# yondonfu/ai-rtc-agent

Measured on NVIDIA H100. Metric: frames/sec at 512x512 SD-Turbo img2img (1-step, stream-batch 1), higher is better.
Workload: dtype f16

## Files before the change

ai-rtc-agent_b200/csrc/capi.cu:

```cuda
#include "../../include/b200sd.h"

#include "attention.cuh"
#include "codec.cuh"
#include "elementwise.cuh"
#include "igemm.cuh"
#include "tconv.cuh"

using namespace b2;

extern "C" {

const char* b2sd_last_error(void) { return b2_last_error(); }
int b2sd_version(void) { return 1; }

static ActView to_view(const b2sd_act_view& v) {
    ActView a;
    a.ptr = reinterpret_cast<const __half*>(v.ptr);
    a.N = v.n; a.H = v.h; a.W = v.w; a.C = v.c; a.ld = v.ld;
    return a;
}

static void to_igemm_desc(const b2sd_igemm_desc* d, IgemmDesc& g) {
    g.nseg = d->nseg;
    for (int s = 0; s < d->nseg && s < IG_MAX_SRC; ++s) {
// ... 7 lines not shown
    g.Nb = d->nb; g.Ho = d->ho; g.Wo = d->wo;
    g.BN = d->bn;
    g.swap = d->swap;
    g.pair = (d->flags & B2SD_IG_PAIR) ? 1 : 0;
    g.splits = d->splits;
    g.partial = nullptr;
    g.dbg_ts = reinterpret_cast<unsigned long long*>(d->partial);
    g.epi.out = reinterpret_cast<__half*>(d->out);
    g.epi.ldc = d->ldc;
    g.epi.colbias = d->colbias;
    g.epi.colbias_bstride = d->colbias_bstride;
    g.epi.res = reinterpret_cast<const __half*>(d->res);
    g.epi.ldr = d->ldr;
    g.epi.acc_scale = d->acc_scale;
    g.epi.res_scale = d->res_scale;
    g.epi.flags = d->flags & (IG_RELU | IG_GEGLU | IG_SILU | IG_PAD0);
    g.epi.n_valid = d->n_valid;
    g.epi.rowstat_out = static_cast<unsigned long long*>(d->rowstat_out);
    g.epi.rowstat_in = static_cast<const unsigned long long*>(d->rowstat_in);
    g.epi.colsum = d->colsum;
    g.epi.ln_inv_c = d->ln_c > 0 ? 1.f / (float)d->ln_c : 0.f;
    g.epi.ln_eps = d->ln_eps;
    g.epi.out2 = reinterpret_cast<__half*>(d->out2);
    g.epi.ld2 = d->ld2;
    g.epi.col2 = d->col2;
}

static b2sd_act_view from_view(const ActView& a) {
    b2sd_act_view v;
    v.ptr = a.ptr;
    v.n = a.N; v.h = a.H; v.w = a.W; v.c = a.C; v.ld = a.ld;
// ... 3 lines not shown
static void fill_plan_info(const IgemmPlan& plan, b2sd_igemm_plan_info* out) {
    out->mode = plan.mode;
    out->swap = plan.p.swap;
    out->bn = plan.p.BN;
    out->splits = plan.splits;
    out->grid_x = (int)plan.grid.x; out->grid_y = (int)plan.grid.y; out->grid_z = (int)plan.grid.z;
    out->num_stages = plan.p.num_stages;
    out->acc_bufs = plan.p.acc_bufs;
    out->total_kb = plan.p.total_kb;
    out->kb_per_split = plan.p.kb_per_split;
    out->tmem_cols = (int)plan.p.tmem_cols;
    out->m_tiles = plan.p.tiles_w * plan.p.tiles_h * plan.p.tiles_n;
    out->smem_bytes = (int64_t)plan.smem;
    out->rows_total = plan.rows_total;
    out->tw = plan.p.tw; out->th = plan.p.th; out->tn = plan.p.tn;
}

}

namespace b2 {
void igemm_record(const IgemmDesc& g, const IgemmPlan* plan, b2sd_igemm_desc* d, b2sd_igemm_plan_info* info) {
    *d = b2sd_igemm_desc{};
    *info = b2sd_igemm_plan_info{};
    d->nseg = g.nseg;
    for (int s = 0; s < g.nseg && s < IG_MAX_SRC; ++s) {
        d->src[s] = from_view(g.src[s]);
        d->ntap[s] = g.ntap[s];
    }
    d->w = g.w;
    d->w_rows = g.w_rows;
// ... 227 lines not shown
```

ai-rtc-agent_b200/csrc/epilogue.cuh:

```cuda
#pragma once
#include "igemm.cuh"
#include "ptx.cuh"
#include "wgmma.cuh"

namespace b2 {

__device__ __forceinline__ float gelu_erf(float x) {
    return 0.5f * x * (1.0f + erff(x * 0.70710678118654752440f));
}

__device__ __forceinline__ float silu_f(float x) { return x / (1.0f + expf(-x)); }

__device__ __forceinline__ void store_half16(__half* dst, const float* v, int nv, bool vec_ok) {
    if (nv == 16 && vec_ok) {
        uint4 u[2];
        __half2* h = reinterpret_cast<__half2*>(u);
#pragma unroll
        for (int i = 0; i < 8; ++i) h[i] = __floats2half2_rn(v[2 * i], v[2 * i + 1]);
        reinterpret_cast<uint4*>(dst)[0] = u[0];
        reinterpret_cast<uint4*>(dst)[1] = u[1];
    } else {
#pragma unroll
        for (int i = 0; i < 16; ++i)
            if (i < nv) dst[i] = __float2half_rn(v[i]);
// ... 112 lines not shown
        *reinterpret_cast<__half2*>(dst) = __floats2half2_rn(x0, x1);
    } else {
        dst[0] = __float2half_rn(x0);
        if (two) dst[1] = __float2half_rn(x1);
    }
}

__device__ __forceinline__ void rowstat_quad(const IgEpilogue& e, const EpiRow& rw, float s1, float s2, int lane) {
    s1 += __shfl_xor_sync(0xffffffffu, s1, 1);
    s2 += __shfl_xor_sync(0xffffffffu, s2, 1);
    s1 += __shfl_xor_sync(0xffffffffu, s1, 2);
    s2 += __shfl_xor_sync(0xffffffffu, s2, 2);
    if ((lane & 3) == 0 && rw.ok) rowstat_add(e, rw.orow, s1, s2);
}

template <int BN, bool SILU = false>
__device__ __forceinline__ void epi_frag(const IgEpilogue& e, const float (&acc)[BN / 2], const EpiRow (&rw)[2], int ntile,
                                         bool ln_fma, int lane) {
    const int q2 = 2 * (lane & 3);
    const bool vec_out = (e.ldc & 1) == 0;
    if (e.flags & IG_GEGLU) {
        constexpr int HALF = BN / 2;
        const int pv0 = ntile * BN, oc0 = ntile * HALF;
#pragma unroll
        for (int j = 0; j < HALF / 8; ++j) {
            const int c = 8 * j + q2;
#pragma unroll
            for (int h = 0; h < 2; ++h) {
                if (!rw[h].ok) continue;
                float v[2];
#pragma unroll
                for (int u = 0; u < 2; ++u) {
                    float a = acc[4 * j + 2 * h + u], g = acc[4 * (j + HALF / 8) + 2 * h + u];
                    const int pv = pv0 + c + u, pg = pv0 + HALF + c + u;
                    if (ln_fma) {
                        const float nmr = -rw[h].mu * rw[h].rstd;
                        a = fmaf(rw[h].rstd, a, fmaf(nmr, e.colsum[pv], e.colbias ? e.colbias[pv] : 0.f));
                        g = fmaf(rw[h].rstd, g, fmaf(nmr, e.colsum[pg], e.colbias ? e.colbias[pg] : 0.f));
                    } else {
                        if (e.colsum) {
                            a = rw[h].rstd * (a - rw[h].mu * e.colsum[pv]);
                            g = rw[h].rstd * (g - rw[h].mu * e.colsum[pg]);
                        }
                        if (e.colbias) {
                            a += e.colbias[pv];
                            g += e.colbias[pg];
                        }
                    }
                    v[u] = a * gelu_erf(g);
                }
                store_half2(e.out + rw[h].orow * e.ldc + oc0 + c, v[0], v[1], true, vec_out);
            }
        }
        return;
    }
    float s1[2] = {0.f, 0.f}, s2[2] = {0.f, 0.f};
#pragma unroll
    for (int j = 0; j < BN / 8; ++j) {
        const int col = ntile * BN + 8 * j + q2;
        if (col >= e.n_valid) continue;
        const bool two = col + 1 < e.n_valid;
        const bool transposed = e.out2 && col >= e.col2;
#pragma unroll
        for (int h = 0; h < 2; ++h) {
            if (!rw[h].ok) continue;
            float x[2] = {acc[4 * j + 2 * h], acc[4 * j + 2 * h + 1]};
// ... 5 lines not shown
                    x[u] = fmaf(rw[h].rstd, x[u], fmaf(nmr, e.colsum[col + u], bp && (u == 0 || two) ? bp[u] : 0.f));
            } else {
                if (e.colsum) {
#pragma unroll
                    for (int u = 0; u < 2; ++u)
                        if (u == 0 || two) x[u] = rw[h].rstd * (x[u] - rw[h].mu * e.colsum[col + u]);
                }
                if (bp) {
                    x[0] += bp[0];
                    if (two) x[1] += bp[1];
                }
                if (e.acc_scale != 1.0f) {
                    x[0] *= e.acc_scale;
                    x[1] *= e.acc_scale;
                }
                if (e.res) {
                    const __half* rp = e.res + rw[h].orow * e.ldr + col;
                    if (two && (e.ldr & 1) == 0) {
                        const float2 f = __half22float2(*reinterpret_cast<const __half2*>(rp));
                        x[0] += e.res_scale * f.x;
                        x[1] += e.res_scale * f.y;
                    } else {
                        x[0] += e.res_scale * __half2float(rp[0]);
                        if (two) x[1] += e.res_scale * __half2float(rp[1]);
                    }
                }
                if (e.flags & IG_RELU) {
                    x[0] = fmaxf(x[0], 0.f);
                    x[1] = fmaxf(x[1], 0.f);
                }
                if (SILU && (e.flags & IG_SILU)) {
// ... 1 lines not shown
                    x[1] = silu_f(x[1]);
                }
            }
            if (transposed) {
                __half* tp = e.out2 + (long)(col - e.col2) * e.ld2 + rw[h].orow;
                tp[0] = __float2half_rn(x[0]);
                if (two) tp[e.ld2] = __float2half_rn(x[1]);
                continue;
            }
            if (e.rowstat_out && !ln_fma) {
                const float r0 = __half2float(__float2half_rn(x[0]));
                const float r1 = two ? __half2float(__float2half_rn(x[1])) : 0.f;
                s1[h] += r0 + r1;
                s2[h] += r0 * r0 + r1 * r1;
            }
            store_half2(e.out + rw[h].orow * e.ldc + col, x[0], x[1], two, vec_out);
        }
    }
    if (e.rowstat_out && !ln_fma) {
        rowstat_quad(e, rw[0], s1[0], s2[0], lane);
        rowstat_quad(e, rw[1], s1[1], s2[1], lane);
    }
}

template <int BN>
__device__ __forceinline__ void frag_to_smem(float* dst, const float (&acc)[BN / 2], int r0, int lane, int c0, int nc, bool colmajor) {
    const int q2 = 2 * (lane & 3);
#pragma unroll
    for (int j = 0; j < BN / 8; ++j) {
        const int c = 8 * j + q2 - c0;
        if (c < 0 || c >= nc) continue;
#pragma unroll
        for (int h = 0; h < 2; ++h) {
            const int r = r0 + 8 * h;
            if (colmajor) {
                dst[c * 128 + r] = acc[4 * j + 2 * h];
                dst[(c + 1) * 128 + r] = acc[4 * j + 2 * h + 1];
// ... 10 lines not shown
```

ai-rtc-agent_b200/csrc/igemm.cu:

```cuda
#include "igemm.cuh"

#include <cudaTypedefs.h>
#include <stdarg.h>
#include <stdio.h>
#include <stdlib.h>
#include <string.h>

#include "epilogue.cuh"
#include "launch.cuh"
#include "ptx.cuh"

namespace b2 {

#ifdef B2_TIMELINE
#define B2_TS(stmt) stmt
#else
#define B2_TS(stmt)
#endif

static thread_local char g_err[1024] = "";
const char* b2_last_error() { return g_err; }
void b2_set_error(const char* fmt, ...) {
    va_list ap;
    va_start(ap, fmt);
// ... 93 lines not shown
#pragma unroll
        for (int s = 0; s < G; ++s) {
            const uint32_t peer = dsmem_map(stg_local, (uint32_t)((s0 + s) * rank_mul + rank_add));
#pragma unroll
            for (int i = 0; i < 4; ++i) v[s][i] = dsmem_ld_f4(peer + (uint32_t)(((cc * 4 + i) * IG_BM + row) * 16));
        }
#pragma unroll
        for (int s = 0; s < G; ++s)
#pragma unroll
            for (int i = 0; i < 4; ++i) {
                acc[4 * i] += v[s][i].x; acc[4 * i + 1] += v[s][i].y; acc[4 * i + 2] += v[s][i].z; acc[4 * i + 3] += v[s][i].w;
            }
    }
}

template <int BN, bool PAIR, bool SILU, bool PAD0 = false>
__device__ __forceinline__ void igemm_body(const IgemmParams& p) {
    extern __shared__ uint8_t smem_raw[];
    uint8_t* smem = reinterpret_cast<uint8_t*>((reinterpret_cast<uintptr_t>(smem_raw) + 1023) &
                                               ~static_cast<uintptr_t>(1023));
    const int warp = threadIdx.x >> 5;
    const int lane = threadIdx.x & 31;
    constexpr uint32_t A_BYTES = IG_BM * IG_BK * 2;
    constexpr uint32_t stage_bytes = A_BYTES + (uint32_t)BN * IG_BK * 2;
    uint64_t* full_bar = reinterpret_cast<uint64_t*>(smem + (size_t)p.num_stages * stage_bytes);
    uint64_t* empty_bar = full_bar + IG_MAX_STAGES;
    const int cr = PAIR ? (int)(blockIdx.x & 1) : 0;
    const int mt_first = (int)blockIdx.x;
    const int mt_step = (int)gridDim.x;
    const int mt_guard = PAIR ? cr : 0;

    const int num_mtiles = p.tiles_w * p.tiles_h * p.tiles_n;
    const int ntile = blockIdx.y;
    const int kb_begin = blockIdx.z * p.kb_per_split;
    const int kb_end = min(p.total_kb, kb_begin + p.kb_per_split);
    [[maybe_unused]] unsigned long long* ts = p.dbg_ts ? p.dbg_ts + ((size_t)(blockIdx.z * gridDim.y + blockIdx.y) * gridDim.x + blockIdx.x) * 8 : nullptr;
    B2_TS(if (ts && threadIdx.x == 0) ts[0] = globaltimer_ns();)

    if (threadIdx.x == IG_CONS) {
        for (int s = 0; s < p.nseg; ++s) tma_prefetch_desc(&p.tmA[s]);
        tma_prefetch_desc(&p.tmB);
        for (int s = 0; s < p.num_stages; ++s) {
            mbar_init(&full_bar[s], 1);
            mbar_init(&empty_bar[s], (PAIR ? 2 : 1) * (IG_CONS / 32));
        }
        fence_mbar_init();
    }
    if (PAIR) {
        cluster_arrive_relaxed();
        cluster_wait();
    }
    __syncthreads();

    pdl_launch_dependents();
    pdl_wait();
    B2_TS(if (ts && threadIdx.x == 0) ts[1] = globaltimer_ns();)

    if (warp == IG_CONS / 32) {
        if (lane == 0) {
// ... 42 lines not shown
                        }
                    }
                    if (++stage == p.num_stages) {
                        stage = 0;
                        phase ^= 1;
                    }
                }
            }
        }
    } else {
        const int wg = warp >> 2;
        const int r0 = wg * 64 + (warp & 3) * 16 + (lane >> 2);
        [[maybe_unused]] const uint32_t peer_empty = PAIR ? dsmem_map(smem_u32(empty_bar), cluster_ctarank() ^ 1u) : 0u;
        const IgEpilogue& e = p.epi;
        const bool ln_fma = e.colsum && !p.swap && !(e.flags & IG_SPLITK) && (e.ldc & 7) == 0 && (e.n_valid & 15) == 0;
        const uint32_t smem_base = smem_u32(smem);
        auto release = [&](int s) {
            if (lane == 0) {
                mbar_arrive(&empty_bar[s]);
                if (PAIR) mbar_arrive_remote(peer_empty + (uint32_t)s * 8u);
            }
        };
        int stage = 0;
        uint32_t phase = 0;
        int it = 0;
        for (int mt = mt_first; mt - mt_guard < num_mtiles; mt += mt_step, ++it) {
            float acc[BN / 2];
#pragma unroll
            for (int i = 0; i < BN / 2; ++i) acc[i] = 0.f;
            int prev = -1;
// ... 5 lines not shown
                const uint64_t db = make_kmajor_sw128_desc(sa + A_BYTES);
#ifdef B2_BOUND_STUDY
                if (p.dbg_mode != 2)
#endif
                {
                    wgmma_fence_regs(acc);
                    wgmma_fence();
#pragma unroll
                    for (int k = 0; k < 4; ++k) Wgmma<BN>::ss(acc, da + 2 * k, db + 2 * k, 1u);
                    wgmma_commit();
                    wgmma_wait<1>();
                    wgmma_fence_regs(acc);
                }
                if (prev >= 0) release(prev);
                prev = stage;
                if (++stage == p.num_stages) {
                    stage = 0;
                    phase ^= 1;
                }
            }
            wgmma_wait<0>();
            wgmma_fence_regs(acc);
            if (prev >= 0) release(prev);
            B2_TS(if (ts && it == 0 && threadIdx.x == 0) ts[4] = globaltimer_ns();)

            const int w0 = (mt % p.tiles_w) * p.tw, h0 = ((mt / p.tiles_w) % p.tiles_h) * p.th;
            const int n0 = (mt / (p.tiles_w * p.tiles_h)) * p.tn;
            if (p.swap || (e.flags & IG_SPLITK)) {
                float* stg = reinterpret_cast<float*>(smem);
                cons_bar_sync();
// ... 9 lines not shown
                        cons_bar_sync();
                    }
                }
            } else {
                EpiRow rw[2];
#pragma unroll
                for (int h = 0; h < 2; ++h) {
                    const int r = r0 + 8 * h;
                    const int wi = r % p.tw, hi = (r / p.tw) % p.th, ni = r / (p.tw * p.th);
                    const int n = n0 + ni, hh = h0 + hi, ww = w0 + wi;
                    rw[h].ok = (ni < p.tn) && (n < p.Nb) && (hh < p.Ho) && (ww < p.Wo);
                    rw[h].orow = ((long)n * p.Ho + hh) * p.Wo + ww;
                    rw[h].b = n;
                    ln_row_stats(e, rw[h].orow, rw[h].ok, rw[h].mu, rw[h].rstd);
                }
                epi_frag<BN, SILU>(e, acc, rw, ntile, ln_fma, lane);
            }
            B2_TS(if (ts && it == 0 && threadIdx.x == 0) ts[5] = globaltimer_ns();)
        }
    }
    if (p.epi.flags & IG_SPLITK) {
        const int mt = blockIdx.x;
        const int w0 = (mt % p.tiles_w) * p.tw, h0 = ((mt / p.tiles_w) % p.tiles_h) * p.th;
        const int n0 = (mt / (p.tiles_w * p.tiles_h)) * p.tn;
        const int splits = (int)gridDim.z;
        const int rk_mul = PAIR ? 2 : 1, rk_add = cr;
        cluster_sync_all();
        B2_TS(if (ts && threadIdx.x == 0) ts[6] = globaltimer_ns();)
        if (warp < IG_CONS / 32 && p.swap) {
            const int rank = (int)cluster_ctarank();
            const int cols_per = BN / splits;
            const int ch = cols_per < SWAP_CH ? cols_per : SWAP_CH;
            const int t = threadIdx.x & (IG_BM - 1);
            const int half = threadIdx.x >> 7;
// ... 56 lines not shown
                    float mu, rstd;
                    ln_row_stats(p.epi, orow, true, mu, rstd);
                    epi_store16<0, 16, float, SILU>(p.epi, acc, n, orow, ntile * BN + cc * 16, mu, rstd);
                }
            }
        }
        B2_TS(if (ts && threadIdx.x == 0) ts[7] = globaltimer_ns();)
        cluster_sync_all();
    }
    if (PAIR) {
        cluster_arrive_relaxed();
        cluster_wait();
    }
}

template <int BN, bool PAIR, bool SILU = false>
__global__ void __launch_bounds__(IG_THREADS, 1) igemm_kernel(const __grid_constant__ IgemmParams p) { igemm_body<BN, PAIR, SILU>(p); }
template <int BN>
__global__ void __launch_bounds__(IG_THREADS, 1) igemm_pad0_kernel(const __grid_constant__ IgemmParams p) { igemm_body<BN, false, false, true>(p); }

using IgemmFn = void (*)(IgemmParams);
template <bool PAIR>
static IgemmFn igemm_fn(int bn) {
    switch (bn) {
#define B2_IG_CASE(N) case N: if constexpr (PAIR && (N % 32)) return nullptr; else return igemm_kernel<N, PAIR>;
        B2_IG_CASE(16) B2_IG_CASE(32) B2_IG_CASE(48) B2_IG_CASE(64) B2_IG_CASE(80) B2_IG_CASE(96) B2_IG_CASE(112) B2_IG_CASE(128)
        B2_IG_CASE(144) B2_IG_CASE(160) B2_IG_CASE(176) B2_IG_CASE(192) B2_IG_CASE(208) B2_IG_CASE(224) B2_IG_CASE(240) B2_IG_CASE(256)
#undef B2_IG_CASE
        default: return nullptr;
    }
}
static IgemmFn igemm_select(int bn, bool pair, bool silu, bool pad0 = false) {
    if (pad0) {
        if (pair || silu) return nullptr;
        switch (bn) {
            case 64: return igemm_pad0_kernel<64>;
            case 128: return igemm_pad0_kernel<128>;
            case 256: return igemm_pad0_kernel<256>;
            default: return nullptr;
        }
    }
    if (!silu) return pair ? igemm_fn<true>(bn) : igemm_fn<false>(bn);
    if (pair) return nullptr;
    switch (bn) {
        case 16: return igemm_kernel<16, false, true>;
        case 32: return igemm_kernel<32, false, true>;
        case 64: return igemm_kernel<64, false, true>;
// ... 9 lines not shown
    cudaDriverEntryPointQueryResult qres;
    cudaError_t err = cudaGetDriverEntryPoint("cuTensorMapEncodeTiled", &p, cudaEnableDefault, &qres);
    if (err != cudaSuccess || qres != cudaDriverEntryPointSuccess || !p) {
        b2_set_error("cudaGetDriverEntryPoint(cuTensorMapEncodeTiled) failed: %s",
                     cudaGetErrorString(err));
        return nullptr;
    }
    fn = reinterpret_cast<PFN_cuTensorMapEncodeTiled_v12000>(p);
    return fn;
}

static thread_local bool g_plan_dry = false;
void igemm_set_dry_run(bool on) { g_plan_dry = on; }

static int encode_act_map(CUtensorMap* m, const ActView& a, int box_c, int box_w, int box_h, int box_n,
                          int estride) {
    if (g_plan_dry) return 0;
    auto enc = get_encode();
    if (!enc) return -1;
    cuuint64_t dims[4] = {(cuuint64_t)a.C, (cuuint64_t)a.W, (cuuint64_t)a.H, (cuuint64_t)a.N};
    cuuint64_t strides[3] = {(cuuint64_t)a.ld * 2, (cuuint64_t)a.W * a.ld * 2,
                             (cuuint64_t)a.H * a.W * a.ld * 2};
    cuuint32_t box[4] = {(cuuint32_t)box_c, (cuuint32_t)box_w, (cuuint32_t)box_h, (cuuint32_t)box_n};
    cuuint32_t es[4] = {1, (cuuint32_t)estride, (cuuint32_t)estride, 1};
    CUresult r = enc(m, CU_TENSOR_MAP_DATA_TYPE_FLOAT16, 4, const_cast<__half*>(a.ptr), dims, strides,
                     box, es, CU_TENSOR_MAP_INTERLEAVE_NONE, CU_TENSOR_MAP_SWIZZLE_128B,
                     CU_TENSOR_MAP_L2_PROMOTION_L2_256B, CU_TENSOR_MAP_FLOAT_OOB_FILL_NONE);
    if (r != CUDA_SUCCESS) {
        b2_set_error("cuTensorMapEncodeTiled(act) failed: %d (ptr %p dims %d,%d,%d,%d ld %d box "
                     "%d,%d,%d,%d es %d)",
                     (int)r, a.ptr, a.C, a.W, a.H, a.N, a.ld, box_c, box_w, box_h, box_n, estride);
        return -1;
    }
    return 0;
}

static int encode_w_map(CUtensorMap* m, const __half* w, int rows, int ld, int box_rows) {
    if (g_plan_dry) return 0;
    auto enc = get_encode();
    if (!enc) return -1;
    cuuint64_t dims[2] = {(cuuint64_t)ld, (cuuint64_t)rows};
// ... 125 lines not shown
            sms = n;
        else
            sms = IG_SMS;
        cudaGetLastError();
    }
    return sms;
}

static int igemm_ctas_per_sm(int bn, bool pair, bool silu, bool pad0) {
    if (g_plan_dry) return 1;
    IgemmFn fn = igemm_select(bn, pair, silu, pad0);
    int n = 0;
    if (fn && cudaOccupancyMaxActiveBlocksPerMultiprocessor(&n, fn, IG_THREADS, 0) == cudaSuccess && n > 0) return n;
    cudaGetLastError();
    return 1;
}

int igemm_plan(const IgemmDesc& d, IgemmPlan* plan) {
    *plan = IgemmPlan{};
    if (d.swap) return plan_swap(d, plan);
    IgemmParams& p = plan->p;
    if (d.nseg < 1 || d.nseg > IG_MAX_SRC) {
        b2_set_error("igemm: bad nseg %d", d.nseg);
        return -1;
    }
    const bool geglu = (d.epi.flags & IG_GEGLU) != 0;
    const int n_gemm = geglu ? d.epi.n_valid * 2 : d.epi.n_valid;
    int BN = d.BN;
    if (BN <= 0) {
        if (n_gemm <= 256 && n_gemm % 16 == 0) BN = n_gemm;
// ... 125 lines not shown
    p.num_stages = stages;
    size_t pipe_bytes = stages * stage_bytes;
    if (splits > 1) {
        const size_t stg = (size_t)BN * IG_BM * 4;
        if (stg > pipe_bytes) {
            stages = (int)((stg + stage_bytes - 1) / stage_bytes);
            if (stages > IG_MAX_STAGES) {
                b2_set_error("igemm: split-K staging does not fit (BN %d)", BN);
                return -1;
            }
            p.num_stages = stages;
            pipe_bytes = stages * stage_bytes;
        }
    }
    plan->smem = pipe_bytes + 1024  + 512 ;
    const int m_tiles = p.tiles_w * p.tiles_h * p.tiles_n;
    int grid_x = m_tiles;
    p.acc_bufs = 1;
    if (will_persist) {
        grid_x = (int)(persist_ctas / n_tiles);
        if (grid_x < 1) grid_x = 1;
        if (grid_x > m_tiles) grid_x = m_tiles;
        p.acc_bufs = 2;
    }
    if (pair) {
        grid_x = (p.acc_bufs == 2 && grid_x > 2) ? (grid_x & ~1) : ((grid_x + 1) & ~1);
    }
    uint32_t cols = 32;
    while (cols < (uint32_t)(BN * p.acc_bufs)) cols <<= 1;
    p.tmem_cols = cols;
    plan->grid = dim3(grid_x, n_tiles, splits);
    plan->mode = pair ? 1 : 0;
    plan->pair = pair ? 1 : 0;
    return 0;
}

int igemm_encode_act_map(CUtensorMap* m, const ActView& a, int box_c, int box_w, int box_h, int box_n, int estride) {
    return encode_act_map(m, a, box_c, box_w, box_h, box_n, estride);
}
int igemm_encode_w_map(CUtensorMap* m, const __half* w, int rows, int ld, int box_rows) { return encode_w_map(m, w, rows, ld, box_rows); }

int igemm_init() {
    static bool attr_set = false;
    if (!attr_set) {
        for (int bn = 16; bn <= 256; bn += 16) {
            for (int pair = 0; pair < 4; ++pair) {
                IgemmFn fn = igemm_select(bn, pair == 1, pair == 2, pair == 3);
                if (!fn) continue;
                cudaError_t e = cudaFuncSetAttribute(fn, cudaFuncAttributeMaxDynamicSharedMemorySize, 227 * 1024);
                if (e != cudaSuccess) {
                    b2_set_error("cudaFuncSetAttribute(igemm BN %d%s): %s", bn, pair ? " pair" : "", cudaGetErrorString(e));
                    return -1;
                }
            }
        }
        if (!get_encode()) return -1;
        attr_set = true;
    }
    return 0;
}

int igemm_launch(const IgemmPlan& plan, cudaStream_t stream) {
    if (igemm_init()) return -1;
    const int cz = plan.splits > 1 ? plan.splits : 1;
    IgemmFn fn = igemm_select(plan.p.BN, plan.pair, (plan.p.epi.flags & IG_SILU) != 0, (plan.p.epi.flags & IG_PAD0) != 0);
    if (!fn) {
        b2_set_error("igemm launch: no kernel for BN %d%s%s%s", plan.p.BN, plan.pair ? " (CTA pair)" : "",
                     (plan.p.epi.flags & IG_SILU) ? " with the SiLU epilogue" : "", (plan.p.epi.flags & IG_PAD0) ? " with tap origin 0" : "");
        return -1;
    }
    cudaError_t e = plan.pair ? launch_kc(fn, plan.grid, dim3(IG_THREADS), plan.smem, stream, 2, cz, plan.p)
                              : launch_k(fn, plan.grid, dim3(IG_THREADS), plan.smem, stream, cz, plan.p);
    if (e != cudaSuccess) {
        b2_set_error("igemm launch: %s", cudaGetErrorString(e));
        return -1;
    }
    return 0;
}

}
// ... 1 lines not shown
```

ai-rtc-agent_b200/csrc/igemm.cuh:

```cuda
#pragma once
#include <cuda.h>
#include <cuda_fp16.h>
#include <cuda_runtime.h>
#include <stdint.h>

namespace b2 {

constexpr int IG_BM = 128;
constexpr int IG_BK = 64;
constexpr int IG_MAX_SRC = 3;
constexpr int IG_MAX_STAGES = 8;
constexpr int IG_CONS = 256;
constexpr int IG_THREADS = IG_CONS + 32;
constexpr int IG_SMS = 132;

enum : int {
    IG_RELU = 1,
    IG_GEGLU = 2,
    IG_SPLITK = 4,
    IG_SILU = 8,
    IG_PAD0 = 16,
};

struct IgEpilogue {
    __half* out;
    int ldc;
    const float* colbias;
    int colbias_bstride;
    const __half* res;
    int ldr;
    float acc_scale;
    float res_scale;
    int flags;
    int n_valid;
    unsigned long long* rowstat_out;
    const unsigned long long* rowstat_in;
    const float* colsum;
    float ln_inv_c, ln_eps;
    __half* out2;
    int ld2, col2;
};

constexpr float IG_STAT_SCALE = 1048576.f;

struct IgemmParams {
    CUtensorMap tmA[IG_MAX_SRC];
    CUtensorMap tmB;
    int seg_ntap[IG_MAX_SRC];
    int seg_cblocks[IG_MAX_SRC];
    int seg_c0[IG_MAX_SRC];
    int nseg;
    int total_kb;
    int kb_per_split;
    int tw, th, tn;
    int tiles_w, tiles_h, tiles_n;
    int Wo, Ho, Nb;
    int stride;
    int BN;
    int num_stages;
    int acc_bufs;
    uint32_t a_bytes;
    uint32_t b_bytes;
    uint32_t tmem_cols;
    unsigned long long* dbg_ts;
    int n_pad;
    int swap;
    int tw_log2, th_log2;
    int dbg_mode;
    IgEpilogue epi;
};

struct ActView {
    const __half* ptr;
    int N, H, W, C;
    int ld;
};

struct IgemmDesc {
    ActView src[IG_MAX_SRC];
    int ntap[IG_MAX_SRC];
    int nseg;
    const __half* w;
    int w_rows;
// ... 40 lines not shown
```

ai-rtc-agent_b200/host/capi.py:

```python
from __future__ import annotations

import ctypes as C
import os

_HERE = os.path.dirname(os.path.abspath(__file__))
LIB_PATH = os.environ.get("B200SD_LIB") or os.path.join(os.path.dirname(_HERE), "libb200sd.so")


class B2Error(RuntimeError):
    pass


class ActView(C.Structure):
    _fields_ = [("ptr", C.c_void_p), ("n", C.c_int), ("h", C.c_int), ("w", C.c_int), ("c", C.c_int),
                ("ld", C.c_int)]


class IgemmDesc(C.Structure):
    _fields_ = [
        ("src", ActView * 3), ("ntap", C.c_int * 3), ("nseg", C.c_int),
        ("w", C.c_void_p), ("w_rows", C.c_int), ("w_ld", C.c_int), ("stride", C.c_int),
        ("nb", C.c_int), ("ho", C.c_int), ("wo", C.c_int),
        ("bn", C.c_int), ("splits", C.c_int), ("partial", C.c_void_p),
        ("out", C.c_void_p), ("ldc", C.c_int),
# ... 1 lines not shown
        ("res", C.c_void_p), ("ldr", C.c_int),
        ("acc_scale", C.c_float), ("res_scale", C.c_float),
        ("flags", C.c_int), ("n_valid", C.c_int), ("swap", C.c_int),
        ("rowstat_out", C.c_void_p), ("rowstat_in", C.c_void_p), ("colsum", C.c_void_p), ("ln_c", C.c_int), ("ln_eps", C.c_float),
        ("out2", C.c_void_p), ("ld2", C.c_int), ("col2", C.c_int),
    ]


class IgemmPlanInfo(C.Structure):
    _fields_ = [
        ("mode", C.c_int), ("swap", C.c_int), ("bn", C.c_int), ("splits", C.c_int),
        ("grid_x", C.c_int), ("grid_y", C.c_int), ("grid_z", C.c_int),
        ("num_stages", C.c_int), ("acc_bufs", C.c_int), ("total_kb", C.c_int), ("kb_per_split", C.c_int),
        ("tmem_cols", C.c_int), ("m_tiles", C.c_int),
        ("smem_bytes", C.c_int64), ("rows_total", C.c_int64),
        ("tw", C.c_int), ("th", C.c_int), ("tn", C.c_int),
    ]


class AttnDesc(C.Structure):
    _fields_ = [
        ("q", C.c_void_p), ("ldq", C.c_int),
        ("k", C.c_void_p), ("ldk", C.c_int), ("k_bstride", C.c_int64), ("k_rows", C.c_int64),
        ("vt", C.c_void_p), ("ldvt", C.c_int), ("vt_bstride", C.c_int64), ("vt_cols", C.c_int64),
        ("out", C.c_void_p), ("ldo", C.c_int),
        ("nb", C.c_int), ("heads", C.c_int), ("sq", C.c_int), ("skv", C.c_int), ("d_real", C.c_int),
        ("dp", C.c_int),
    ]


class GroupNormArgs(C.Structure):
# ... 89 lines not shown
        ("vae", C.c_int), ("vae_scaling_factor", C.c_float),
    ]


class LoraFactor(C.Structure):
    _fields_ = [("key", C.c_char_p), ("up", C.c_void_p), ("down", C.c_void_p), ("rank", C.c_int), ("dtype", C.c_int),
                ("scale", C.c_float)]


IN_U8_NHWC, IN_F32_NCHW, IN_F16_NCHW = 0, 1, 2
OUT_U8_NCHW, OUT_F16_NCHW = 0, 1
IG_RELU = 1
IG_GEGLU = 2
IG_SILU = 8
IG_PAD0 = 16
SC_IN_U8, SC_IN_TANH3, SC_OUT_RELU, SC_OUT_SILU, SC_IN_OFFSET = 1, 2, 4, 32, 64
CONTROL_FRAME, CONTROL_HED = 0, 1
COND_PROMPT, COND_TIME = 0, 1
VAE_TINY, VAE_KL = 0, 1
IG_TCONV = 64
IG_PAIR = 128

_lib = None


def lib() -> C.CDLL:
    global _lib
    if _lib is None:
        if not os.path.exists(LIB_PATH):
            raise B2Error(f"{LIB_PATH} not found: build it with `make -C ai-rtc-agent_b200/csrc` "
# ... 91 lines not shown
```

ai-rtc-agent_b200/host/ops.py:

```python
from __future__ import annotations

import ctypes as C
from typing import Optional, Sequence, Tuple

import torch

from . import capi


_SCRATCH = {}


def pack_conv_weight(w_oihw: torch.Tensor) -> torch.Tensor:
    o, i, kh, kw = w_oihw.shape
    return w_oihw.permute(0, 2, 3, 1).reshape(o, kh * kw * i).contiguous().to(torch.float16)


def _pitch(t: torch.Tensor) -> int:
    n, h, w, _ = t.shape
    return t.stride(2) if w > 1 or (h == 1 and n == 1) else (t.stride(1) if h > 1 else t.stride(0))


def _view(t: torch.Tensor) -> capi.ActView:
    assert t.dtype == torch.float16 and t.is_cuda and t.dim() == 4
    n, h, w, c = t.shape
    assert t.stride(3) == 1 and t.stride(2) % 8 == 0
    ld = t.stride(2)
    assert t.stride(1) == w * ld and t.stride(0) == h * w * ld, "NHWC view must be dense in n,h,w"
    return capi.ActView(t.data_ptr(), n, h, w, c, ld)


def igemm(srcs: Sequence[Tuple[torch.Tensor, int]], w: torch.Tensor, out: torch.Tensor, *,
          stride: int = 1, colbias: Optional[torch.Tensor] = None, res: Optional[torch.Tensor] = None,
          acc_scale: float = 1.0, res_scale: float = 1.0, relu: bool = False, geglu: bool = False, silu: bool = False,
          bn: int = 0, splits: int = 1, n_valid: Optional[int] = None, timeline: Optional[torch.Tensor] = None, swap: bool = False,
          tconv: bool = False, pair: bool = False, pad0: bool = False,
          rowstat_out: Optional[torch.Tensor] = None, rowstat_in: Optional[torch.Tensor] = None,
          colsum: Optional[torch.Tensor] = None, ln_c: int = 0, ln_eps: float = 1e-5,
          out2: Optional[torch.Tensor] = None, col2: int = 0) -> torch.Tensor:
    d = _igemm_desc(srcs, w, out, stride=stride, colbias=colbias, res=res, acc_scale=acc_scale, res_scale=res_scale, relu=relu,
                    geglu=geglu, silu=silu, bn=bn, splits=splits, n_valid=n_valid, timeline=timeline, swap=swap, tconv=tconv, pair=pair,
                    pad0=pad0,
                    rowstat_out=rowstat_out, rowstat_in=rowstat_in, colsum=colsum, ln_c=ln_c, ln_eps=ln_eps, out2=out2, col2=col2)
    capi.check(capi.lib().b2sd_op_igemm(C.byref(d), capi.current_stream_ptr()), "b2sd_op_igemm")
    return out


def igemm_engine_plan(srcs, w, out, *, autotile: int = 1, allow_swap: bool = True, **kw) -> capi.IgemmPlanInfo:
    d = _igemm_desc(srcs, w, out, **kw)
    info = capi.IgemmPlanInfo()
    capi.check(capi.lib().b2sd_igemm_plan_dry(C.byref(d), autotile, int(allow_swap), C.byref(info)), "b2sd_igemm_plan_dry")
    return info


def _igemm_desc(srcs, w, out, *, stride=1, colbias=None, res=None, acc_scale=1.0, res_scale=1.0, relu=False, geglu=False,
                silu=False, bn=0, splits=1, n_valid=None, timeline=None, swap=False, tconv=False, pair=False, pad0=False, rowstat_out=None,
                rowstat_in=None, colsum=None, ln_c=0, ln_eps=1e-5, out2=None, col2=0) -> capi.IgemmDesc:
    d = capi.IgemmDesc()
    d.nseg = len(srcs)
    for i, (t, ntap) in enumerate(srcs):
        d.src[i] = _view(t)
        d.ntap[i] = ntap
    assert w.dtype == torch.float16 and w.is_contiguous()
    d.w, d.w_rows, d.w_ld = w.data_ptr(), w.shape[0], w.shape[1]
    d.stride = stride
    nb, ho, wo, _ = out.shape
    d.nb, d.ho, d.wo = nb, ho, wo
    d.bn, d.splits = bn, splits
    d.swap = int(swap)
    d.out, d.ldc = out.data_ptr(), _pitch(out)
    nv = n_valid if n_valid is not None else out.shape[3]
    d.n_valid = nv
    if timeline is not None:
        d.partial = timeline.data_ptr()
    if colbias is not None:
        assert colbias.dtype == torch.float32 and colbias.is_contiguous()
        d.colbias = colbias.data_ptr()
        d.colbias_bstride = colbias.shape[1] if colbias.dim() == 2 and colbias.shape[0] > 1 else 0
    if res is not None:
        assert res.dtype == torch.float16
        d.res, d.ldr = res.data_ptr(), _pitch(res)
    d.acc_scale, d.res_scale = acc_scale, res_scale
    d.flags = (capi.IG_RELU if relu else 0) | (capi.IG_GEGLU if geglu else 0) | (capi.IG_TCONV if tconv else 0) | (capi.IG_PAIR if pair else 0) \
        | (capi.IG_SILU if silu else 0) | (capi.IG_PAD0 if pad0 else 0)
    if rowstat_out is not None:
        assert rowstat_out.dtype == torch.int64 and rowstat_out.is_contiguous()
        d.rowstat_out = rowstat_out.data_ptr()
    if rowstat_in is not None:
        assert rowstat_in.dtype == torch.int64 and colsum is not None and colsum.dtype == torch.float32 and ln_c > 0
        d.rowstat_in, d.colsum, d.ln_c, d.ln_eps = rowstat_in.data_ptr(), colsum.data_ptr(), ln_c, ln_eps
    if out2 is not None:
        assert out2.dtype == torch.float16 and out2.dim() == 2 and out2.stride(1) == 1
        d.out2, d.ld2, d.col2 = out2.data_ptr(), out2.stride(0), col2
    return d


def _sp():
    return capi.current_stream_ptr()

# ... 105 lines not shown
```

include/b200sd.h:

```cpp
#ifndef B200SD_H
#define B200SD_H

#include <stdint.h>

#ifdef __cplusplus
extern "C" {
#endif

const char* b2sd_last_error(void);
int b2sd_version(void);


typedef struct {
    const void* ptr;
    int n, h, w, c;
    int ld;
} b2sd_act_view;

enum {
    B2SD_IG_RELU = 1,
    B2SD_IG_GEGLU = 2,
    B2SD_IG_SILU = 8,
    B2SD_IG_PAD0 = 16,
    B2SD_IG_TCONV = 64,
    B2SD_IG_PAIR = 128
};

typedef struct {
    b2sd_act_view src[3];
    int ntap[3];
    int nseg;
    const void* w;
    int w_rows, w_ld;
    int stride;
    int nb, ho, wo;
    int bn;
    int splits;
    void* partial;
// ... 17 lines not shown
} b2sd_igemm_desc;

int b2sd_op_igemm(const b2sd_igemm_desc* d, void* stream);

typedef struct {
    int mode;
    int swap, bn, splits;
    int grid_x, grid_y, grid_z;
    int num_stages;
    int acc_bufs;
    int total_kb, kb_per_split;
    int tmem_cols;
    int m_tiles;
    int64_t smem_bytes, rows_total;
    int tw, th, tn;
} b2sd_igemm_plan_info;
int b2sd_igemm_plan_dry(const b2sd_igemm_desc* d, int autotile, int allow_swap, b2sd_igemm_plan_info* out);

int b2sd_groupnorm_plan_dry(int ca, int cb, int groups, int hw, int* cluster, int* threads, int* pixels_per_cta);
uint64_t b2sd_igemm_partial_floats(int splits, int64_t rows_total, int n_valid);

typedef struct {
    const void* q; int ldq;
    const void* k; int ldk; int64_t k_bstride; int64_t k_rows;
    const void* vt; int ldvt; int64_t vt_bstride; int64_t vt_cols;
    void* out; int ldo;
    int nb, heads, sq, skv, d_real, dp;
} b2sd_attn_desc;
int b2sd_op_attention(const b2sd_attn_desc* d, void* stream);

// ... 180 lines not shown
```

Baseline: 197.6.

## Stage igemm epilogue through swizzled smem with TMA residual prefetch and store

Adds a staged epilogue to the implicit-GEMM kernel. At the first k-block the residual tile is prefetched into a 64B-swizzled shared-memory buffer by TMA. Results are then written to that buffer and sent out as bulk TMA stores, replacing per-thread scattered global half2 loads and stores. This needs extra shared memory, which can lower stages or occupancy, and more kernel template instantiations. Staging is on by default and is skipped for split-K, SiLU, pad0, and misaligned outputs.

Result: faster. 205.8 (median of 6 runs) (+4.2%).

```diff
diff --git a/ai-rtc-agent_b200/csrc/capi.cu b/ai-rtc-agent_b200/csrc/capi.cu
--- a/ai-rtc-agent_b200/csrc/capi.cu
+++ b/ai-rtc-agent_b200/csrc/capi.cu
@@ -45,7 +45,7 @@
     g.epi.ldr = d->ldr;
     g.epi.acc_scale = d->acc_scale;
     g.epi.res_scale = d->res_scale;
-    g.epi.flags = d->flags & (IG_RELU | IG_GEGLU | IG_SILU | IG_PAD0);
+    g.epi.flags = d->flags & (IG_RELU | IG_GEGLU | IG_SILU | IG_PAD0 | IG_NO_STAGE);
     g.epi.n_valid = d->n_valid;
     g.epi.rowstat_out = static_cast<unsigned long long*>(d->rowstat_out);
     g.epi.rowstat_in = static_cast<const unsigned long long*>(d->rowstat_in);
@@ -79,6 +79,7 @@
     out->smem_bytes = (int64_t)plan.smem;
     out->rows_total = plan.rows_total;
     out->tw = plan.p.tw; out->th = plan.p.th; out->tn = plan.p.tn;
+    out->staged = plan.p.staged;
 }
 
 }
diff --git a/ai-rtc-agent_b200/csrc/epilogue.cuh b/ai-rtc-agent_b200/csrc/epilogue.cuh
--- a/ai-rtc-agent_b200/csrc/epilogue.cuh
+++ b/ai-rtc-agent_b200/csrc/epilogue.cuh
@@ -150,11 +150,14 @@
     if ((lane & 3) == 0 && rw.ok) rowstat_add(e, rw.orow, s1, s2);
 }
 
-template <int BN, bool SILU = false>
+template <int BN, bool SILU = false, bool STAGED = false>
 __device__ __forceinline__ void epi_frag(const IgEpilogue& e, const float (&acc)[BN / 2], const EpiRow (&rw)[2], int ntile,
-                                         bool ln_fma, int lane) {
+                                         bool ln_fma, int lane, uint8_t* stg = nullptr) {
     const int q2 = 2 * (lane & 3);
     const bool vec_out = (e.ldc & 1) == 0;
+    auto sp = [&](int h, int j) {
+        return reinterpret_cast<__half2*>(stg + h * (8 * 64) + (j >> 2) * IG_STG_BOX + (((j & 3) ^ (lane >> 3)) << 4));
+    };
     if (e.flags & IG_GEGLU) {
         constexpr int HALF = BN / 2;
         const int pv0 = ntile * BN, oc0 = ntile * HALF;
@@ -185,7 +188,8 @@
                     }
                     v[u] = a * gelu_erf(g);
                 }
-                store_half2(e.out + rw[h].orow * e.ldc + oc0 + c, v[0], v[1], true, vec_out);
+                if constexpr (STAGED) *sp(h, j) = __floats2half2_rn(v[0], v[1]);
+                else store_half2(e.out + rw[h].orow * e.ldc + oc0 + c, v[0], v[1], true, vec_out);
             }
         }
         return;
@@ -221,7 +225,11 @@
                     x[0] *= e.acc_scale;
                     x[1] *= e.acc_scale;
                 }
-                if (e.res) {
+                if (STAGED && e.res) {
+                    const float2 f = __half22float2(*sp(h, j));
+                    x[0] += e.res_scale * f.x;
+                    x[1] += e.res_scale * f.y;
+                } else if (e.res) {
                     const __half* rp = e.res + rw[h].orow * e.ldr + col;
                     if (two && (e.ldr & 1) == 0) {
                         const float2 f = __half22float2(*reinterpret_cast<const __half2*>(rp));
@@ -253,13 +261,18 @@
                 s1[h] += r0 + r1;
                 s2[h] += r0 * r0 + r1 * r1;
             }
-            store_half2(e.out + rw[h].orow * e.ldc + col, x[0], x[1], two, vec_out);
+            if constexpr (STAGED) *sp(h, j) = __floats2half2_rn(x[0], x[1]);
+            else store_half2(e.out + rw[h].orow * e.ldc + col, x[0], x[1], two, vec_out);
         }
     }
     if (e.rowstat_out && !ln_fma) {
         rowstat_quad(e, rw[0], s1[0], s2[0], lane);
         rowstat_quad(e, rw[1], s1[1], s2[1], lane);
     }
+}
+
+__device__ __forceinline__ uint8_t* stg_thread(uint8_t* stg, int warp, int lane) {
+    return stg + ((warp & 3) * 16 + (lane >> 2)) * 64 + 4 * (lane & 3);
 }
 
 template <int BN>
diff --git a/ai-rtc-agent_b200/csrc/igemm.cu b/ai-rtc-agent_b200/csrc/igemm.cu
--- a/ai-rtc-agent_b200/csrc/igemm.cu
+++ b/ai-rtc-agent_b200/csrc/igemm.cu
@@ -131,17 +131,19 @@
     }
 }
 
-template <int BN, bool PAIR, bool SILU, bool PAD0 = false>
+template <int BN, bool PAIR, bool SILU, bool PAD0 = false, bool STAGED = false>
 __device__ __forceinline__ void igemm_body(const IgemmParams& p) {
     extern __shared__ uint8_t smem_raw[];
-    uint8_t* smem = reinterpret_cast<uint8_t*>((reinterpret_cast<uintptr_t>(smem_raw) + 1023) &
-                                               ~static_cast<uintptr_t>(1023));
+    uint8_t* smem = smem_raw + ((1024u - (smem_u32(smem_raw) & 1023u)) & 1023u);
     const int warp = threadIdx.x >> 5;
     const int lane = threadIdx.x & 31;
     constexpr uint32_t A_BYTES = IG_BM * IG_BK * 2;
     constexpr uint32_t stage_bytes = A_BYTES + (uint32_t)BN * IG_BK * 2;
-    uint64_t* full_bar = reinterpret_cast<uint64_t*>(smem + (size_t)p.num_stages * stage_bytes);
+    const uint32_t stg_bytes = STAGED ? (uint32_t)p.stg_boxes * IG_STG_BOX : 0u;
+    uint8_t* stg_base = smem + (size_t)p.num_stages * stage_bytes;
+    uint64_t* full_bar = reinterpret_cast<uint64_t*>(stg_base + 2 * stg_bytes);
     uint64_t* empty_bar = full_bar + IG_MAX_STAGES;
+    uint64_t* r_full = empty_bar + IG_MAX_STAGES;
     const int cr = PAIR ? (int)(blockIdx.x & 1) : 0;
     const int mt_first = (int)blockIdx.x;
     const int mt_step = (int)gridDim.x;
@@ -160,6 +162,12 @@
         for (int s = 0; s < p.num_stages; ++s) {
             mbar_init(&full_bar[s], 1);
             mbar_init(&empty_bar[s], (PAIR ? 2 : 1) * (IG_CONS / 32));
+        }
+        if (stg_bytes) {
+            tma_prefetch_desc(&p.tmO);
+            if (p.epi.res) tma_prefetch_desc(&p.tmR);
+            mbar_init(&r_full[0], 1);
+            mbar_init(&r_full[1], 1);
         }
         fence_mbar_init();
     }
@@ -232,6 +240,11 @@
         [[maybe_unused]] const uint32_t peer_empty = PAIR ? dsmem_map(smem_u32(empty_bar), cluster_ctarank() ^ 1u) : 0u;
         const IgEpilogue& e = p.epi;
         const bool ln_fma = e.colsum && !p.swap && !(e.flags & IG_SPLITK) && (e.ldc & 7) == 0 && (e.n_valid & 15) == 0;
+        const bool staged = stg_bytes && !(e.out2 && (ntile + 1) * BN > e.col2);
+        const bool leader = (threadIdx.x & 127) == 0;
+        const bool load_res = e.res && !(e.flags & IG_GEGLU) && !ln_fma;
+        const int ow = (e.flags & IG_GEGLU) ? BN / 2 : BN;
+        uint8_t* stg = stg_base + wg * stg_bytes;
         const uint32_t smem_base = smem_u32(smem);
         auto release = [&](int s) {
             if (lane == 0) {
@@ -267,6 +280,19 @@
                 }
                 if (prev >= 0) release(prev);
                 prev = stage;
+                if (staged && leader && kb == kb_begin) {
+                    const int w0 = (mt % p.tiles_w) * p.tw, h0 = ((mt / p.tiles_w) % p.tiles_h) * p.th;
+                    const int n0 = (mt / (p.tiles_w * p.tiles_h)) * p.tn;
+                    bulk_wait_group_read<0>();
+                    if (load_res) {
+                        mbar_expect_tx(&r_full[wg], stg_bytes);
+                        for (int b = 0; b < p.stg_boxes; ++b)
+                            tma_load_4d(stg + b * IG_STG_BOX, &p.tmR, &r_full[wg], ntile * ow + 32 * b, w0 + wg * p.stg_dw,
+                                        h0 + wg * p.stg_dh, n0 + wg * p.stg_dn);
+                    } else {
+                        mbar_arrive(&r_full[wg]);
+                    }
+                }
                 if (++stage == p.num_stages) {
                     stage = 0;
                     phase ^= 1;
@@ -306,10 +332,24 @@
                     rw[h].b = n;
                     ln_row_stats(e, rw[h].orow, rw[h].ok, rw[h].mu, rw[h].rstd);
                 }
-                epi_frag<BN, SILU>(e, acc, rw, ntile, ln_fma, lane);
+                if (staged) {
+                    mbar_wait(&r_full[wg], (uint32_t)it & 1u);
+                    epi_frag<BN, SILU, true>(e, acc, rw, ntile, ln_fma, lane, stg_thread(stg, warp, lane));
+                    fence_proxy_async_smem();
+                    named_bar_sync(2 + wg, 128);
+                    if (leader) {
+                        for (int b = 0; b < p.stg_boxes; ++b)
+                            tma_store_4d(&p.tmO, stg + b * IG_STG_BOX, ntile * ow + 32 * b, w0 + wg * p.stg_dw, h0 + wg * p.stg_dh,
+                                         n0 + wg * p.stg_dn);
+                        bulk_commit_group();
+                    }
+                } else {
+                    epi_frag<BN, SILU>(e, acc, rw, ntile, ln_fma, lane);
+                }
             }
             B2_TS(if (ts && it == 0 && threadIdx.x == 0) ts[5] = globaltimer_ns();)
         }
+        if (staged && leader) bulk_wait_group<0>();
     }
     if (p.epi.flags & IG_SPLITK) {
         const int mt = blockIdx.x;
@@ -396,23 +436,29 @@
     }
 }
 
-template <int BN, bool PAIR, bool SILU = false>
-__global__ void __launch_bounds__(IG_THREADS, 1) igemm_kernel(const __grid_constant__ IgemmParams p) { igemm_body<BN, PAIR, SILU>(p); }
+template <int BN, bool PAIR, bool SILU = false, bool STAGED = false>
+__global__ void __launch_bounds__(IG_THREADS, 1) igemm_kernel(const __grid_constant__ IgemmParams p) {
+    igemm_body<BN, PAIR, SILU, false, STAGED>(p);
+}
 template <int BN>
 __global__ void __launch_bounds__(IG_THREADS, 1) igemm_pad0_kernel(const __grid_constant__ IgemmParams p) { igemm_body<BN, false, false, true>(p); }
 
 using IgemmFn = void (*)(IgemmParams);
-template <bool PAIR>
+template <bool PAIR, bool STAGED = false>
 static IgemmFn igemm_fn(int bn) {
     switch (bn) {
-#define B2_IG_CASE(N) case N: if constexpr (PAIR && (N % 32)) return nullptr; else return igemm_kernel<N, PAIR>;
+#define B2_IG_CASE(N) case N: if constexpr ((PAIR || STAGED) && (N % 32)) return nullptr; else return igemm_kernel<N, PAIR, false, STAGED>;
         B2_IG_CASE(16) B2_IG_CASE(32) B2_IG_CASE(48) B2_IG_CASE(64) B2_IG_CASE(80) B2_IG_CASE(96) B2_IG_CASE(112) B2_IG_CASE(128)
         B2_IG_CASE(144) B2_IG_CASE(160) B2_IG_CASE(176) B2_IG_CASE(192) B2_IG_CASE(208) B2_IG_CASE(224) B2_IG_CASE(240) B2_IG_CASE(256)
 #undef B2_IG_CASE
         default: return nullptr;
     }
 }
-static IgemmFn igemm_select(int bn, bool pair, bool silu, bool pad0 = false) {
+static IgemmFn igemm_select(int bn, bool pair, bool silu, bool pad0 = false, bool staged = false) {
+    if (staged) {
+        if (silu || pad0) return nullptr;
+        return pair ? igemm_fn<true, true>(bn) : igemm_fn<false, true>(bn);
+    }
     if (pad0) {
         if (pair || silu) return nullptr;
         switch (bn) {
@@ -452,7 +498,7 @@
 void igemm_set_dry_run(bool on) { g_plan_dry = on; }
 
 static int encode_act_map(CUtensorMap* m, const ActView& a, int box_c, int box_w, int box_h, int box_n,
-                          int estride) {
+                          int estride, CUtensorMapSwizzle swz = CU_TENSOR_MAP_SWIZZLE_128B) {
     if (g_plan_dry) return 0;
     auto enc = get_encode();
     if (!enc) return -1;
@@ -462,7 +508,7 @@
     cuuint32_t box[4] = {(cuuint32_t)box_c, (cuuint32_t)box_w, (cuuint32_t)box_h, (cuuint32_t)box_n};
     cuuint32_t es[4] = {1, (cuuint32_t)estride, (cuuint32_t)estride, 1};
     CUresult r = enc(m, CU_TENSOR_MAP_DATA_TYPE_FLOAT16, 4, const_cast<__half*>(a.ptr), dims, strides,
-                     box, es, CU_TENSOR_MAP_INTERLEAVE_NONE, CU_TENSOR_MAP_SWIZZLE_128B,
+                     box, es, CU_TENSOR_MAP_INTERLEAVE_NONE, swz,
                      CU_TENSOR_MAP_L2_PROMOTION_L2_256B, CU_TENSOR_MAP_FLOAT_OOB_FILL_NONE);
     if (r != CUDA_SUCCESS) {
         b2_set_error("cuTensorMapEncodeTiled(act) failed: %d (ptr %p dims %d,%d,%d,%d ld %d box "
@@ -618,6 +664,37 @@
     if (fn && cudaOccupancyMaxActiveBlocksPerMultiprocessor(&n, fn, IG_THREADS, 0) == cudaSuccess && n > 0) return n;
     cudaGetLastError();
     return 1;
+}
+
+static int plan_staging(const IgemmDesc& d, bool geglu, bool two_per_sm, IgemmPlan* plan) {
+    IgemmParams& p = plan->p;
+    const IgEpilogue& e = p.epi;
+    p.staged = 0;
+    const int ow = geglu ? p.BN / 2 : p.BN;
+    const int rows = p.tw * p.th;
+    int box_w = p.tw, box_h = 0, box_n = 0;
+    p.stg_dw = p.stg_dh = p.stg_dn = 0;
+    if (64 % rows == 0) { box_h = p.th; box_n = 64 / rows; p.stg_dn = box_n; }
+    else if (rows == IG_BM && 64 % p.tw == 0) { box_h = 64 / p.tw; box_n = 1; p.stg_dh = box_h; }
+    else if (rows == IG_BM && p.tw == IG_BM) { box_w = 64; box_h = 1; box_n = 1; p.stg_dw = 64; }
+    auto a16 = [](const void* q) { return (reinterpret_cast<uintptr_t>(q) & 15) == 0; };
+    const int ch = e.out2 && e.col2 < e.n_valid ? e.col2 : e.n_valid;
+    const bool tma_ok = a16(e.out) && (e.ldc & 7) == 0 && ch > 0 && (ch & 7) == 0 && (!e.res || (a16(e.res) && (e.ldr & 7) == 0));
+    const size_t stg_bytes = (size_t)(ow / 32) * IG_STG_BOX;
+    const size_t smem = plan->smem + 2 * stg_bytes;
+    if (plan->splits > 1 || (e.flags & (IG_NO_STAGE | IG_PAD0 | IG_SILU)) || ow % 32 != 0 || !box_h || !tma_ok ||
+        smem > (size_t)(two_per_sm ? 113 : 227) * 1024)
+        return 0;
+    const ActView out{e.out, d.Nb, d.Ho, d.Wo, ch, e.ldc};
+    if (encode_act_map(&p.tmO, out, 32, box_w, box_h, box_n, 1, CU_TENSOR_MAP_SWIZZLE_64B)) return -1;
+    if (e.res && !geglu) {
+        const ActView res{e.res, d.Nb, d.Ho, d.Wo, ch, e.ldr};
+        if (encode_act_map(&p.tmR, res, 32, box_w, box_h, box_n, 1, CU_TENSOR_MAP_SWIZZLE_64B)) return -1;
+    }
+    p.staged = 1;
+    p.stg_boxes = ow / 32;
+    plan->smem = smem;
+    return 0;
 }
 
 int igemm_plan(const IgemmDesc& d, IgemmPlan* plan) {
@@ -773,6 +850,7 @@
         }
     }
     plan->smem = pipe_bytes + 1024  + 512 ;
+    if (int rc = plan_staging(d, geglu, per_sm >= 2 && total_ctas > b2_device_sms(), plan)) return rc;
     const int m_tiles = p.tiles_w * p.tiles_h * p.tiles_n;
     int grid_x = m_tiles;
     p.acc_bufs = 1;
@@ -803,8 +881,8 @@
     static bool attr_set = false;
     if (!attr_set) {
         for (int bn = 16; bn <= 256; bn += 16) {
-            for (int pair = 0; pair < 4; ++pair) {
-                IgemmFn fn = igemm_select(bn, pair == 1, pair == 2, pair == 3);
+            for (int pair = 0; pair < 6; ++pair) {
+                IgemmFn fn = igemm_select(bn, pair == 1 || pair == 5, pair == 2, pair == 3, pair >= 4);
                 if (!fn) continue;
                 cudaError_t e = cudaFuncSetAttribute(fn, cudaFuncAttributeMaxDynamicSharedMemorySize, 227 * 1024);
                 if (e != cudaSuccess) {
@@ -822,7 +900,8 @@
 int igemm_launch(const IgemmPlan& plan, cudaStream_t stream) {
     if (igemm_init()) return -1;
     const int cz = plan.splits > 1 ? plan.splits : 1;
-    IgemmFn fn = igemm_select(plan.p.BN, plan.pair, (plan.p.epi.flags & IG_SILU) != 0, (plan.p.epi.flags & IG_PAD0) != 0);
+    IgemmFn fn = igemm_select(plan.p.BN, plan.pair, (plan.p.epi.flags & IG_SILU) != 0, (plan.p.epi.flags & IG_PAD0) != 0,
+                              plan.p.staged != 0);
     if (!fn) {
         b2_set_error("igemm launch: no kernel for BN %d%s%s%s", plan.p.BN, plan.pair ? " (CTA pair)" : "",
                      (plan.p.epi.flags & IG_SILU) ? " with the SiLU epilogue" : "", (plan.p.epi.flags & IG_PAD0) ? " with tap origin 0" : "");
diff --git a/ai-rtc-agent_b200/csrc/igemm.cuh b/ai-rtc-agent_b200/csrc/igemm.cuh
--- a/ai-rtc-agent_b200/csrc/igemm.cuh
+++ b/ai-rtc-agent_b200/csrc/igemm.cuh
@@ -20,7 +20,9 @@
     IG_SPLITK = 4,
     IG_SILU = 8,
     IG_PAD0 = 16,
+    IG_NO_STAGE = 32,
 };
+constexpr uint32_t IG_STG_BOX = 64 * 32 * 2;
 
 struct IgEpilogue {
     __half* out;
@@ -46,6 +48,7 @@
 struct IgemmParams {
     CUtensorMap tmA[IG_MAX_SRC];
     CUtensorMap tmB;
+    CUtensorMap tmO, tmR;
     int seg_ntap[IG_MAX_SRC];
     int seg_cblocks[IG_MAX_SRC];
     int seg_c0[IG_MAX_SRC];
@@ -67,6 +70,9 @@
     int swap;
     int tw_log2, th_log2;
     int dbg_mode;
+    int staged;
+    int stg_boxes;
+    int stg_dw, stg_dh, stg_dn;
     IgEpilogue epi;
 };
 
diff --git a/ai-rtc-agent_b200/host/capi.py b/ai-rtc-agent_b200/host/capi.py
--- a/ai-rtc-agent_b200/host/capi.py
+++ b/ai-rtc-agent_b200/host/capi.py
@@ -39,7 +39,7 @@
         ("num_stages", C.c_int), ("acc_bufs", C.c_int), ("total_kb", C.c_int), ("kb_per_split", C.c_int),
         ("tmem_cols", C.c_int), ("m_tiles", C.c_int),
         ("smem_bytes", C.c_int64), ("rows_total", C.c_int64),
-        ("tw", C.c_int), ("th", C.c_int), ("tn", C.c_int),
+        ("tw", C.c_int), ("th", C.c_int), ("tn", C.c_int), ("staged", C.c_int),
     ]
 
 
@@ -159,6 +159,7 @@
 IG_GEGLU = 2
 IG_SILU = 8
 IG_PAD0 = 16
+IG_NO_STAGE = 32
 SC_IN_U8, SC_IN_TANH3, SC_OUT_RELU, SC_OUT_SILU, SC_IN_OFFSET = 1, 2, 4, 32, 64
 CONTROL_FRAME, CONTROL_HED = 0, 1
 COND_PROMPT, COND_TIME = 0, 1
diff --git a/ai-rtc-agent_b200/host/ops.py b/ai-rtc-agent_b200/host/ops.py
--- a/ai-rtc-agent_b200/host/ops.py
+++ b/ai-rtc-agent_b200/host/ops.py
@@ -37,10 +37,10 @@
           tconv: bool = False, pair: bool = False, pad0: bool = False,
           rowstat_out: Optional[torch.Tensor] = None, rowstat_in: Optional[torch.Tensor] = None,
           colsum: Optional[torch.Tensor] = None, ln_c: int = 0, ln_eps: float = 1e-5,
-          out2: Optional[torch.Tensor] = None, col2: int = 0) -> torch.Tensor:
+          out2: Optional[torch.Tensor] = None, col2: int = 0, staged: bool = True) -> torch.Tensor:
     d = _igemm_desc(srcs, w, out, stride=stride, colbias=colbias, res=res, acc_scale=acc_scale, res_scale=res_scale, relu=relu,
                     geglu=geglu, silu=silu, bn=bn, splits=splits, n_valid=n_valid, timeline=timeline, swap=swap, tconv=tconv, pair=pair,
-                    pad0=pad0,
+                    pad0=pad0, staged=staged,
                     rowstat_out=rowstat_out, rowstat_in=rowstat_in, colsum=colsum, ln_c=ln_c, ln_eps=ln_eps, out2=out2, col2=col2)
     capi.check(capi.lib().b2sd_op_igemm(C.byref(d), capi.current_stream_ptr()), "b2sd_op_igemm")
     return out
@@ -55,7 +55,7 @@
 
 def _igemm_desc(srcs, w, out, *, stride=1, colbias=None, res=None, acc_scale=1.0, res_scale=1.0, relu=False, geglu=False,
                 silu=False, bn=0, splits=1, n_valid=None, timeline=None, swap=False, tconv=False, pair=False, pad0=False, rowstat_out=None,
-                rowstat_in=None, colsum=None, ln_c=0, ln_eps=1e-5, out2=None, col2=0) -> capi.IgemmDesc:
+                rowstat_in=None, colsum=None, ln_c=0, ln_eps=1e-5, out2=None, col2=0, staged=True) -> capi.IgemmDesc:
     d = capi.IgemmDesc()
     d.nseg = len(srcs)
     for i, (t, ntap) in enumerate(srcs):
@@ -82,7 +82,7 @@
         d.res, d.ldr = res.data_ptr(), _pitch(res)
     d.acc_scale, d.res_scale = acc_scale, res_scale
     d.flags = (capi.IG_RELU if relu else 0) | (capi.IG_GEGLU if geglu else 0) | (capi.IG_TCONV if tconv else 0) | (capi.IG_PAIR if pair else 0) \
-        | (capi.IG_SILU if silu else 0) | (capi.IG_PAD0 if pad0 else 0)
+        | (capi.IG_SILU if silu else 0) | (capi.IG_PAD0 if pad0 else 0) | (0 if staged else capi.IG_NO_STAGE)
     if rowstat_out is not None:
         assert rowstat_out.dtype == torch.int64 and rowstat_out.is_contiguous()
         d.rowstat_out = rowstat_out.data_ptr()
diff --git a/include/b200sd.h b/include/b200sd.h
--- a/include/b200sd.h
+++ b/include/b200sd.h
@@ -22,6 +22,7 @@
     B2SD_IG_GEGLU = 2,
     B2SD_IG_SILU = 8,
     B2SD_IG_PAD0 = 16,
+    B2SD_IG_NO_STAGE = 32,
     B2SD_IG_TCONV = 64,
     B2SD_IG_PAIR = 128
 };
@@ -69,6 +70,7 @@
     int m_tiles;
     int64_t smem_bytes, rows_total;
     int tw, th, tn;
+    int staged;
 } b2sd_igemm_plan_info;
 int b2sd_igemm_plan_dry(const b2sd_igemm_desc* d, int autotile, int allow_swap, b2sd_igemm_plan_info* out);
 
```
